# bc-computing/fantoch

Hardware: AMD Instinct MI355X
Metric: executed cmds/sec (node) for batched Atlas/EPaxos sims; % of HBM roofline (higher is better)
Workload: dtype u32

## Files before the change

fantoch_amd/csrc/sim_wave.hip:

```cpp
#include <hip/hip_runtime.h>
#include <stdint.h>

#include <algorithm>
#include <cstdio>
#include <cstring>
#include <vector>

#include "fantoch_amd.h"
#include "fx_internal.h"
#include "fx_synth.h"
#include "fx_wave.h"

namespace fx {
namespace sim {

constexpr uint32_t NMAX = FX_SIM_MAX_N;
constexpr uint32_t CMAX = 32;
constexpr uint32_t KMAX = 2;
constexpr uint32_t VMAX = 16;
constexpr uint32_t FMAX = 12;
constexpr uint32_t RDMAX = 16;
constexpr uint32_t HC_BINS = 64;
constexpr uint32_t HD_BINS = 224;
constexpr uint32_t HMAX = 2;
constexpr uint32_t NONE = 0xFFFFFFFFu;
constexpr uint32_t LNIL = 0xFFFFu;
constexpr uint32_t PT_SEQ = 0, PT_FAST = 8, PT_SLOW = 16, PT_EXEC = 24, PT_OCC = 32, PT_WAIT = 48;

#ifdef FX_SIM_PROFILE
#define PROF_T0() const uint64_t prof_t0_ = __builtin_amdgcn_s_memtime()
#define PROF_ADD(cat) prof[cat] += __builtin_amdgcn_s_memtime() - prof_t0_
#else
#define PROF_T0() (void)0
#define PROF_ADD(cat) (void)0
#endif

enum : uint32_t { M_COLLECT = 0, M_COLLECT_ACK = 1, M_COMMIT = 2, M_CONSENSUS = 3, M_CONSENSUS_ACK = 4,
                  M_COMMIT_DOT = 5, M_GC = 6, M_STABLE = 7,
                  M_STORE = 8, M_STORE_ACK = 9, M_COMMIT_BASIC = 10,
                  M_SUBMIT = 15  };
enum : uint32_t { ST_START = 0, ST_PAYLOAD = 1, ST_COLLECT = 2, ST_COMMIT = 3 };
enum : uint32_t { PH_IDLE = 0, PH_DFS = 1, PH_TRY = 2, PH_CHECK = 3 };

constexpr uint32_t SL_CLIENT = 0,
    SL_IDX = 1, SL_KEYS = 2, SL_PST = 3,
    SL_MASKS = 5, SL_CNT = 6, SL_COLLECT = 7;


struct Geo {
  uint32_t n, C, K, W, R, L, NP, ncli_keys, rt, rc, rdm;
  uint32_t amax, vmax, sl_value, sl_ack, slotw;
  uint32_t off_pool, off_free, off_gct, off_gcc, off_gcr, off_slot, off_kd, off_frame, off_wl, off_hist, words;
};

__host__ __device__ constexpr uint32_t cmin(uint32_t a, uint32_t b) { return a < b ? a : b; }
__host__ __device__ constexpr uint32_t cmax(uint32_t a, uint32_t b) { return a > b ? a : b; }

__host__ __device__ constexpr bool geo_make(uint32_t n, uint32_t C, uint32_t K, uint32_t pool, uint32_t ring,
                                            uint32_t wslots, Geo& g) {
  if (n < 2 || n > NMAX) return false;
  if (C < 1 || C > CMAX) return false;
  g.n = n;
  g.C = C;
  g.K = K;
  const uint32_t cpr = (C + n - 1) / n;
  g.W = wslots ? wslots : (n > 5 && C <= 8 ? 32u : cmin(64u, 8u * C));
  if (g.W > 256u) return false;
  g.R = ring ? ring : cmin(4096u, cmax(16u * n * cpr, n > 5 ? 192u : 0u));
  if (g.R > 65534u) return false;
  g.NP = n * (n - 1);
  g.L = g.NP + n + 2 * C;
  if (g.L > 64 * HMAX) return false;
  g.ncli_keys = pool + C + 1;
  g.amax = 2 * g.K;
  g.vmax = cmin(VMAX, g.K * (n + 1));
  g.sl_value = SL_COLLECT + g.K;
  g.sl_ack = g.sl_value + g.vmax;
  g.slotw = g.sl_ack + n * g.amax;
  if (n * g.amax > 64 || g.slotw > 64) return false;
  uint32_t o = 0;
  g.off_pool = o; o += g.R * 4;
  g.off_free = o; o += g.R;
  g.rt = 4;
  while (g.rt < 4 * cpr && g.rt < 64) g.rt <<= 1;
  if (g.W > 64u) g.rt = cmax(g.rt, 32u);
  g.rc = g.rt / 2;
  g.off_gct = o; o += n * n * g.rt * 2;
  g.off_gcc = o; o += n * n * g.rc * 2;
  if (g.R >= n * n) {
    g.off_gcr = g.off_pool;
  } else {
    g.off_gcr = o; o += n * n * 4;
  }
  g.off_slot = o; o += g.W * g.slotw;
  g.off_kd = o; o += n * g.ncli_keys;
  g.rdm = cmin(RDMAX, C);
  g.off_frame = o; o += FMAX * g.rdm;
  g.off_wl = o; o += 68;
  g.off_hist = o; o += HD_BINS;
  g.words = (o + 3) & ~3u;
  return true;
}
__host__ __device__ constexpr Geo geo_fixed(uint32_t n, uint32_t C) {
  Geo g{};
  geo_make(n, C, 1, 1, 0, 0, g);
  return g;
}

constexpr uint32_t FANY = 0xFFu;
struct GeoRT {
  static constexpr bool fixed = false;
  static constexpr uint32_t proto = 0xFFu, fc = FANY, xp_lanes = 0;
  Geo g;
};
template <uint32_t PR, uint32_t N, uint32_t F, uint32_t CC>
struct GeoCT {
  static constexpr bool fixed = true;
#ifdef FX_XSWAP
  static constexpr uint32_t proto = PR, fc = F, xp_lanes = 0;
#else
  static constexpr uint32_t proto = PR, fc = F, xp_lanes = 64u / N;
#endif
  static constexpr Geo g = geo_fixed(N, CC);
};

struct SimArgs {
  const fx_sim_spec* specs;
  uint32_t instances;
  Geo g;
  const uint16_t* ping;
  const uint8_t* rank;
  uint32_t RP;
  uint32_t exec_cap, lat_cap, max_events, sim_exec_notif;
  uint32_t* executed;
  uint32_t* executed_len;
  uint32_t* latency_log;
  unsigned long long* lat_hist;
  uint32_t lat_bins;
  unsigned long long* chain_hist;
  uint32_t chain_bins;
  unsigned long long* delay_hist;
  uint32_t delay_bins;
  unsigned long long* stats;
  uint32_t* err;
  uint32_t* dot_client;
};

typedef __attribute__((address_space(4))) const SimArgs KSimArgs;
__device__ __forceinline__ KSimArgs* kargs() {
  KSimArgs* p = (KSimArgs*)__builtin_amdgcn_kernarg_segment_ptr();
  asm volatile("" : "+s"(p));
  return p;
}
__device__ __forceinline__ uint32_t vdiv(uint32_t x) {
  uint32_t r;
  asm("v_mov_b32 %0, %1" : "=v"(r) : "v"(x));
  return r;
}

template <uint32_t N>
__device__ __forceinline__ uint32_t rsel(const uint32_t (&a)[N], uint32_t i) {
  uint32_t r = 0;
#pragma unroll
  for (uint32_t k = 0; k < N; ++k) r = (i == k) ? a[k] : r;
  return r;
}
template <uint32_t N>
__device__ __forceinline__ void rput(uint32_t (&a)[N], uint32_t i, uint32_t v) {
#pragma unroll
  for (uint32_t k = 0; k < N; ++k) a[k] = (i == k) ? v : a[k];
}

__device__ __forceinline__ uint32_t tid(uint32_t t) { return t & 127u; }
__device__ __forceinline__ uint32_t tlow(uint32_t t) { return (t >> 7) & 127u; }
__device__ __forceinline__ uint32_t tep(uint32_t t) { return t >> 14; }
__device__ __forceinline__ uint32_t tmk(uint32_t id, uint32_t low, uint32_t ep) { return id | (low << 7) | (ep << 14); }
constexpr uint32_t EPOCH_MAX = 0xFFFFu;

template <uint32_t HM, uint32_t DS, uint32_t NX, class GP>
struct Sim : GP {
  using GP::g;
  uint32_t lid_;
  __device__ __forceinline__ uint32_t lidv() const {
    uint32_t x = lid_;
    asm volatile("" : "+v"(x));
    return x;
  }
  uint32_t* lds;
  uint32_t protocol, n, f, synod_f, fq, wq;
  enum : uint32_t { P_SEED = 0, P_RNG = 2, P_GC = 4, P_EN = 5, P_CMDS = 6, P_CONFLICT = 7, P_POOL = 8, P_EXTRA = 9,
                    P_HAS_EXTRA = 10, P_FINAL = 11, P_CDONE = 12, P_ERRSITE = 13, P_INST = 14,
                    P_F = 15, P_FQ = 16, P_SYNOD_F = 17, P_PROTO = 18, P_OFF_FRAME = 19, P_RDM = 20 };
  uint32_t pv = 0;
  __device__ __forceinline__ uint32_t prm(uint32_t k) const {
    uint32_t r;
    asm volatile("s_nop 1\n\tv_readlane_b32 %0, %1, %2\n\ts_nop 4" : "=s"(r) : "v"(pv), "i"(k));
    return r;
  }
  __device__ __forceinline__ uint64_t prm64(uint32_t k) const {
    return (uint64_t)prm(k) | ((uint64_t)prm(k + 1) << 32);
  }
  __device__ __forceinline__ void prm_set(uint32_t k, uint32_t x) {
    if (lidv() == k) pv = x;
  }
  enum : uint32_t { LG_EXEC = 0, LG_DOTC = 8, LG_LAT = 32 };
  uint64_t lgb = 0;
  uint32_t lgc = 0;
  __device__ __forceinline__ void logs_init(const SimArgs& a, uint32_t inst) {
    const uint32_t l = lidv();
    const bool ex = l < n, dc = (l >= LG_DOTC) & (l - LG_DOTC < n), lt = (l >= LG_LAT) & (l - LG_LAT < g.C);
    const uint64_t prow = (uint64_t)inst * n + (l & 7u), crow = (uint64_t)inst * g.C + (l & 31u);
    const uint64_t be = (uint64_t)a.executed, bd = (uint64_t)a.dot_client, bl = (uint64_t)a.latency_log;
    uint64_t b = 0;
    uint32_t c = 0;
    b = (ex & (be != 0)) ? be + prow * a.exec_cap * 4u : b;
    b = (dc & (bd != 0)) ? bd + prow * a.exec_cap * 4u : b;
    b = (lt & (bl != 0)) ? bl + crow * a.lat_cap * 4u : b;
    c = (ex | dc) ? a.exec_cap : c;
    c = lt ? a.lat_cap : c;
    lgb = b;
    lgc = b != 0 ? c : 0u;
  }
  __device__ __forceinline__ void log_put(uint32_t l, uint32_t table, uint32_t k, uint32_t i, uint32_t v) {
    typedef __attribute__((address_space(1))) uint32_t gu32;
    if ((l - table == k) & (i < lgc)) *(gu32*)(lgb + (uint64_t)i * 4u) = v;
  }
  __device__ __forceinline__ uint32_t proto_() const { if constexpr (GP::fixed) return protocol; else return prm(P_PROTO); }
  __device__ __forceinline__ uint32_t f_() const { if constexpr (GP::fixed) return f; else return prm(P_F); }
  __device__ __forceinline__ uint32_t fq_() const { if constexpr (GP::fixed) return fq; else return prm(P_FQ); }
  __device__ __forceinline__ uint32_t synod_f_() const { if constexpr (GP::fixed) return synod_f; else return prm(P_SYNOD_F); }
  uint32_t C;
  uint32_t err = 0;
  __device__ __forceinline__ void fail_cap(uint32_t line) {
    if (!err) prm_set(P_ERRSITE, line);
    err = FX_ERR_SIM_CAPACITY;
  }
  __device__ __forceinline__ void fail_late(uint32_t line) {
    if (!err) prm_set(P_ERRSITE, line);
    err = FX_ERR_SIM_LATE;
  }
  uint32_t now = 0;
  uint32_t seq = 0;
  uint32_t events = 0;
  uint64_t trace, deps_total, lat_sum;
  uint32_t hcv = 0, hlk = 0, hlc = 0;
  bool done = false, in_extra = false;

  uint32_t ht[HM], hs[HM];
  uint32_t gf = 0, gw = 0, gnt = 0, glk = 0, gkm = 0, gnc = 0;
  uint32_t pt = 0, pq = 0;
  uint32_t ca = 0, cb = 0, cd = 0;
  uint32_t dpq = 0;
  uint32_t frw = 0, frd = 0;
  uint32_t rhv = 0xFFFFFFFFu;
  uint32_t nfree = 0;
  uint32_t sdv[DS];
  uint32_t ecf = 0, ecw = 0;

  uint32_t xdot[NX], xrec[NX], xwait[NX];
  uint32_t sdot, srec, swait, stl, sfr;
  static constexpr bool XSL = GP::xp_lanes != 0;
  uint32_t frow;
  uint64_t occ, wmask, tmask;
  static constexpr uint32_t XPL = GP::xp_lanes;
  uint64_t pmask = ~0ull;
  uint32_t xk, epoch, nwl, phase, root, idc, nfr, missing, fv, fdi, fnc, in_try, emitted, xp;
#ifdef FX_SIM_PROFILE
  uint64_t prof[32] = {};
#endif

  __device__ __forceinline__ uint32_t& W(uint32_t i) { return lds[i]; }
  __device__ __forceinline__ uint32_t& msg(uint32_t e, uint32_t w) {
    return lds[g.off_pool + e * 4 + w];
  }
  __device__ __forceinline__ uint32_t* gct(uint32_t p, uint32_t s) { return &lds[g.off_gct + (p * g.n + s) * g.rt * 2]; }
  __device__ __forceinline__ uint32_t* gcc(uint32_t p, uint32_t s) { return &lds[g.off_gcc + (p * g.n + s) * g.rc * 2]; }
  __device__ __forceinline__ uint32_t* gcr(uint32_t p, uint32_t s) { return &lds[g.off_gcr + (p * g.n + s) * 4]; }
  __device__ __forceinline__ uint32_t slot_find(uint32_t d) const {
    uint32_t r = NONE;
#pragma unroll
    for (uint32_t k = 0; k < DS; ++k) {
      const uint64_t m = bal(sdv[k] == d && d != 0u);
      if (m && r == NONE) r = k * 64u + ctz64(m);
    }
    return r;
  }
  __device__ __forceinline__ void slot_set(uint32_t sl, uint32_t d) {
    const uint32_t l = lidv();
#pragma unroll
    for (uint32_t k = 0; k < DS; ++k) sdv[k] = (((sl >> 6) == k) & (l == (sl & 63u))) ? d : sdv[k];
  }
  __device__ __forceinline__ uint32_t slot_alloc() const {
#pragma unroll
    for (uint32_t k = 0; k < DS; ++k) {
      const uint32_t lo = k * 64u;
      if (lo >= g.W) break;
      const uint64_t pool = g.W - lo >= 64u ? ~0ull : ((1ull << (g.W - lo)) - 1ull);
      const uint64_t fre = ~bal(sdv[k] != 0u) & pool;
      if (fre) return lo + ctz64(fre);
    }
    return NONE;
  }
  __device__ __forceinline__ uint32_t& S(uint32_t sl, uint32_t w) { return lds[g.off_slot + sl * g.slotw + w]; }
  __device__ __forceinline__ uint32_t& kd(uint32_t p, uint32_t key) { return lds[g.off_kd + p * g.ncli_keys + key]; }
  __device__ __forceinline__ uint32_t rdm_() const { if constexpr (GP::fixed) return g.rdm; else return prm(P_RDM); }
  __device__ __forceinline__ uint32_t& FRR(uint32_t fi, uint32_t r) {
    if constexpr (GP::fixed) return lds[g.off_frame + fi * g.rdm + r];
    else return lds[prm(P_OFF_FRAME) + fi * prm(P_RDM) + r];
  }
  __device__ __forceinline__ uint32_t& wl(uint32_t i) { return lds[g.off_wl + i]; }
  __device__ __forceinline__ void hist_chain(uint32_t v) {
    const uint32_t l = lidv();
    if (v < HC_BINS) {
      hcv += l == v ? 1u : 0u;
    } else if (l == 0) {
      KSimArgs* k = kargs();
      if (k->chain_hist) atomicAdd(&k->chain_hist[min(v, k->chain_bins - 1u)], 1ull);
    }
  }
  __device__ __forceinline__ void hist_lat(uint32_t region, uint32_t lat) {
    const uint32_t key = (region << 24) | min(lat, 0xFFFFFFu);
    const uint32_t h = (key * 2654435761u) >> 26;
    const uint32_t k = rl(hlk, h);
    const uint32_t l = lidv();
    if ((k == key + 1u) | (k == 0)) {
      hlk = l == h ? key + 1u : hlk;
      hlc += l == h ? 1u : 0u;
    } else {
      flush_lat(key, 1u);
    }
  }
  __device__ __forceinline__ void flush_lat(uint32_t key, uint32_t cnt) {
    if (lidv() == 0) {
      KSimArgs* k = kargs();
      const uint32_t lat = key & 0xFFFFFFu, bins = k->lat_bins;
      if (k->lat_hist) atomicAdd(&k->lat_hist[(key >> 24) * bins + min(lat, bins - 1u)], (unsigned long long)cnt);
    }
  }
  __device__ __forceinline__ void hist_delay(uint32_t v) {
#ifdef FX_ABL_HIST
    return;
#endif
    const uint32_t l = lidv();
    if (v < HD_BINS) {
      const uint32_t cnt = lds[g.off_hist + v];
      put(lds[g.off_hist + v], cnt + 1u);
    } else if (l == 0) {
      KSimArgs* k = kargs();
      if (k->delay_hist) atomicAdd(&k->delay_hist[min(v, k->delay_bins - 1u)], 1ull);
    }
  }
// ... 496 lines not shown
      if (cl[e * 2] <= x) {
        v = cl[e * 2 + 1];
        return true;
      }
    }
    v = 0;
    return nc <= g.rc;
  }

  __device__ __forceinline__ uint32_t gc_next_after(uint32_t x, uint32_t& pair) {
    const uint32_t gc_ms = prm(P_GC);
    const uint32_t tick = (x / gc_ms + 1u) * gc_ms;
    uint32_t tv = NONE;
    const uint32_t p = lidv() >> 3, q = lidv() & 7u;
    if (p < n && q < n && p != q) {
      const uint32_t d = dpq;
      tv = x < gc_ms + d ? gc_ms + d : ((x - d) / gc_ms + 1u) * gc_ms + d;
    }
    uint32_t tmin = tv;
    for (uint32_t o = 1; o < 64; o <<= 1) tmin = min(tmin, (uint32_t)__shfl_xor((int)tmin, (int)o));
    tmin = uni(tmin);
    if (tick <= tmin) {
      pair = NONE;
      return tick;
    }
    pair = ctz64(bal(tv == tmin));
    return tmin;
  }

  __device__ __forceinline__ void gc_finish(uint32_t tc, uint32_t pair, unsigned long long* st) {
    const uint32_t gc_ms = prm(P_GC);
    if (gc_lane(lidv() >> 3)) {
      uint32_t* r = gcr(lidv() >> 3, lidv() & 7u);
      r[0] = gf;
      r[1] = gnt;
      r[2] = gkm;
      r[3] = gnc;
    }
    for (uint32_t q = 0; q < n; ++q) {
      uint32_t m = 0;
      const bool pl = lidv() < n && lidv() != q;
      const uint32_t dq = gather(dpq, (lidv() * 8u + q) & 63u);
      if (pl) {
        const uint32_t d = dq;
        if (tc > d) m = (tc - d - 1u) / gc_ms;
        if (pair == lidv() * 8u + q && tc >= d + gc_ms && (tc - d) % gc_ms == 0) ++m;
      }
      uint32_t stable = 0;
      if (!bal(pl && m == 0)) {
        uint32_t tl = pl ? m * gc_ms + dq : 0u;
        for (uint32_t o = 1; o < 64; o <<= 1) tl = max(tl, (uint32_t)__shfl_xor((int)tl, (int)o));
        tl = uni(tl);
        uint32_t cur = 0;
        bool ok = true;
        if (lidv() < n) ok = gc_value_at(q, lidv(), tl, cur);
        for (uint32_t p = 0; p < n; ++p) {
          if (p == q) continue;
          const uint32_t kl = rl(m, p) - 1u;
          uint32_t v = 0;
          if (lidv() < n) {
            ok = ok && gc_tick_value(p, lidv(), kl, v);
            cur = min(cur, v);
          }
        }
        if (bal(lidv() < n && !ok)) fail_cap(__LINE__);
        for (uint32_t s2 = 0; s2 < n; ++s2) stable += rl(cur, s2);
      }
      if (st && lidv() == 0) st[FX_SIM_STAT_STABLE + q] = stable;
    }
  }

  __device__ __forceinline__ bool mine(uint64_t m) const {
    return mine(m, lidv());
  }
  __device__ __forceinline__ static bool mine(uint64_t m, uint32_t l) {
    const uint32_t half = l < 32u ? (uint32_t)m : (uint32_t)(m >> 32);
    return (half >> (l & 31u)) & 1u;
  }
  __device__ __forceinline__ uint32_t vcount_of(uint32_t d) { return uni(S(slot_find(d), SL_CNT)) & 0xFFu; }
  __device__ __forceinline__ uint32_t value_at(uint32_t d, uint32_t j) { return uni(S(slot_find(d), g.sl_value + j)); }

  __device__ __forceinline__ void x_load(uint32_t p) {
    xp = p;
    root = idc = nfr = missing = fv = fdi = fnc = in_try = emitted = nwl = 0;
    stl = 0;
    if constexpr (!XSL) sfr = 0;
    frow = 0;
    epoch = 1;
    if constexpr (XPL != 0) {
      pmask = ((1ull << XPL) - 1ull) << (p * XPL);
      occ = bal(sdot != 0u) & pmask;
      wmask = bal(swait != 0u) & pmask;
    } else {
      sdot = rsel(xdot, p); srec = rsel(xrec, p); swait = rsel(xwait, p);
      occ = (uint64_t)rl(pt, PT_OCC + p) | ((uint64_t)rl(pt, PT_OCC + 8u + p) << 32);
      wmask = (uint64_t)rl(pt, PT_WAIT + p) | ((uint64_t)rl(pt, PT_WAIT + 8u + p) << 32);
    }
    xk = rl(pt, PT_EXEC + p);
    tmask = 0;
    phase = PH_IDLE;
  }
  __device__ __forceinline__ void x_store() {
    const uint32_t p = xp;
    if constexpr (XPL != 0) {
      lset(pt, PT_EXEC + p, xk);
      return;
    }
    rput(xdot, p, sdot); rput(xrec, p, srec); rput(xwait, p, swait);
    const uint32_t l = lidv();
    const uint32_t k = (l & 7u) == p ? l >> 3 : NONE;
    pt = k == PT_OCC / 8u ? (uint32_t)occ : pt;
    pt = k == PT_OCC / 8u + 1u ? (uint32_t)(occ >> 32) : pt;
    pt = k == PT_WAIT / 8u ? (uint32_t)wmask : pt;
    pt = k == PT_WAIT / 8u + 1u ? (uint32_t)(wmask >> 32) : pt;
    pt = k == PT_EXEC / 8u ? xk : pt;
  }

  __device__ __forceinline__ bool contains_v(uint32_t d) const {
    const uint32_t si = (d >> FX_SEQ_BITS) - 1u;
    const uint32_t ln = (xp * 8u + si) & 63u;
    const uint32_t fr = gather(ecf, ln), w = gather(ecw, ln);
    const uint32_t sq = d & FX_SEQ_MASK, off = sq - fr - 1u;
    return (si < n) & ((sq <= fr) | ((off < 32u) & (((w >> (off & 31u)) & 1u) != 0u)));
  }
  __device__ __forceinline__ bool contains_u(uint32_t d) const {
    const uint32_t si = (d >> FX_SEQ_BITS) - 1u;
    if (si >= n) return false;
    const uint32_t fr = rl(ecf, xp * 8u + si), w = rl(ecw, xp * 8u + si);
    const uint32_t sq = d & FX_SEQ_MASK, off = sq - fr - 1u;
    return sq <= fr || (off < 32u && ((w >> off) & 1u));
  }
  __device__ __forceinline__ void clk_add(uint32_t d) {
    const uint32_t l = lidv();
    const uint32_t si = (d >> FX_SEQ_BITS) - 1u, sq = d & FX_SEQ_MASK;
    const uint32_t own = si < n ? xp * 8u + si : NONE;
    const uint32_t off = ((l == own) & (sq > ecf)) ? sq - ecf - 1u : NONE;
    if (bal(off + 1u > 32u)) fail_cap(__LINE__);
    ecw |= off - 1u < 31u ? 1u << (off & 31u) : 0u;
    const bool adv = off == 0u;
    const uint32_t win = ecw >> 1;
    const uint32_t ones = __builtin_ctz(~win);
    ecf = adv ? ecf + 1u + ones : ecf;
    ecw = adv ? win >> ones : ecw;
    if (si >= n) err = FX_ERR_DOT_RANGE;
  }
  __device__ __forceinline__ int find(uint32_t d) const {
    const uint64_t m = bal(mine(occ) & (sdot == d));
    return m ? (int)ctz64(m) : -1;
  }
  __device__ __forceinline__ void new_epoch() {
    epoch = epoch + 1;
    if (epoch > EPOCH_MAX) {
      stl = mine(occ) ? tmk(tid(stl), tlow(stl), 0) : stl;
      epoch = 1;
    }
  }

  __device__ __forceinline__ void on_execute(uint32_t d, uint32_t start) {
    const uint32_t sl = slot_find(d);
    if (sl == NONE) { fail_late(__LINE__); return; }
    on_execute_slot(d, start, sl);
  }
  __device__ __forceinline__ void on_execute_slot(uint32_t d, uint32_t start, uint32_t sl) {
    const uint32_t row = slot_row(sl);
    on_execute_at(d, start, sl, rl(row, SL_CLIENT), (rl(row, SL_CNT) >> 20) & 3u, rl(row, SL_MASKS));
  }
  __device__ __forceinline__ void on_execute_at(uint32_t d, uint32_t start, uint32_t sl, uint32_t c, uint32_t nk,
                                                uint32_t masks) {
    const uint32_t p = xp;
    log_put(lidv(), LG_EXEC, p, xk, d);
    ++xk;
    const uint32_t delay = now - start;
    hist_delay(delay);
    if ((rl(ca, c) & 0xFFu) == p) {
      const uint32_t pend = rl(cb, 32u + c);
      if (pend < nk) { fail_late(__LINE__); return; }
      lset(cb, 32u + c, pend - nk);
      if (pend == nk) {
        const uint32_t w = fw_(), nr = (w >> 20) & 31u;
        if (nr >= rdm_()) { fail_cap(__LINE__); return; }
        put(FRR(nfrm - 1, nr), c);
        fw_set(w + (1u << 20));
      }
    }
    if (((masks >> 24) & 0xFFu) + 1u == n) {
      slot_set(sl, 0u);
    } else {
      put(S(sl, SL_MASKS), masks + (1u << 24));
    }
  }

  __device__ __forceinline__ void emit_one(uint32_t d, uint32_t start, uint32_t sl, uint32_t c, uint32_t nk, uint32_t masks) {
    hist_chain(1u);
    clk_add(d);
    on_execute_at(d, start, sl, c, nk, masks);
  }

  __device__ __forceinline__ int insert_vertex(uint32_t d, uint32_t dsl) {
    const uint64_t fre = ~occ & pmask;
    if (!fre) { fail_cap(__LINE__); return -1; }
    const uint32_t sl = ctz64(fre);
    const bool me = lidv() == sl;
    sdot = me ? d : sdot;
    srec = me ? now : srec;
    swait = me ? 0u : swait;
    stl = me ? 0u : stl;
    if constexpr (XSL) sfr = me ? dsl << 16 : sfr;
    occ |= 1ull << sl;
    return (int)sl;
  }

  __device__ __forceinline__ void frame_vertex(uint32_t v) {
    fv = v;
    if constexpr (XSL) {
      frow = slot_row(rl(sfr, v) >> 16);
      fnc = rl(frow, SL_CNT) & 0xFFu;
    } else {
      fnc = vcount_of(rl(sdot, v));
    }
  }
  __device__ __forceinline__ void dfs_start(uint32_t r, bool intry) {
    root = r;
    in_try = intry;
    emitted = 0;
    missing = 0;
    idc = 1;
    const uint32_t tr = rl(stl, r);
    stl = lidv() == r ? tmk(1, 1, tep(tr)) : stl;
    nfr = 0;
    fdi = 0;
    frame_vertex(r);
    phase = PH_DFS;
  }

  __device__ __forceinline__ void save_scc() {
    const uint32_t idv = tid(rl(stl, fv));
    const uint32_t l = lidv();
    const uint32_t myid = tid(stl);
    const bool mem = mine(occ, l) & (myid >= idv);
    const uint64_t mm = bal(mem);
    const uint32_t cnt = pop64(mm);
    if (nwl + cnt > 65u) { fail_cap(__LINE__); return; }
    hist_chain(cnt);
    uint32_t rank = 0;
    for (uint64_t m = mm; m; m &= m - 1) rank += rl(sdot, ctz64(m)) < sdot ? 1u : 0u;
    for (uint32_t r = 0; r < cnt; ++r) {
      const uint32_t lr = ctz64(bal(mem & (rank == r)));
      const uint32_t d = rl(sdot, lr);
      const uint32_t st = rl(srec, lr);
      put(wl(nwl + r), d);
      clk_add(d);
      if constexpr (XSL) on_execute_slot(d, st, rl(sfr, lr) >> 16);
      else on_execute(d, st);
      if (err) return;
    }
    nwl += cnt;
    if constexpr (XPL != 0) {
      sdot = mem ? 0u : sdot;
      swait = mem ? 0u : swait;
    }
    occ &= ~mm;
    wmask &= ~mm;
    tmask &= ~mm;
    emitted = 1;
  }

  __device__ __forceinline__ void dfs_finish() {
    const bool mark = in_try && missing != 0 && !emitted;
    const uint32_t l = lidv();
    const uint32_t myid = tid(stl);
    stl = (mine(occ, l) & (myid != 0)) ? tmk(0, 0, mark ? epoch : tep(stl)) : stl;
    if (missing) {
      swait = l == root ? missing : swait;
      wmask |= 1ull << root;
    }
    if (in_try) {
      if (!missing || emitted) new_epoch();
      phase = PH_TRY;
    } else {
      phase = PH_CHECK;
    }
  }

  __device__ __forceinline__ void dfs_iter() {
    const uint32_t l = lidv();
    if (fdi < fnc) {
      const uint32_t vd = rl(sdot, fv);
      const uint32_t dep = XSL ? rl(frow, g.sl_value + fdi) : value_at(vd, fdi);
      ++fdi;
      if (dep == vd || contains_u(dep)) return;
      const int x = find(dep);
      if (x < 0) {
        missing = dep;
        dfs_finish();
        return;
      }
      const uint32_t tx = rl(stl, (uint32_t)x);
      if (tid(tx) == 0) {
        ++idc;
        if (idc > 127u) { fail_cap(__LINE__); return; }
        stl = l == (uint32_t)x ? tmk(idc, idc, tep(tx)) : stl;
        sfr = l == nfr ? (XSL ? sfr & 0xFFFF0000u : 0u) | fv | (fdi << 8) : sfr;
        ++nfr;
        fdi = 0;
        frame_vertex((uint32_t)x);
      } else {
        const uint32_t tv = rl(stl, fv);
        stl = ((tid(tx) < tlow(tv)) & (l == fv)) ? tmk(tid(tv), tid(tx), tep(tv)) : stl;
      }
    } else {
      const uint32_t tv = rl(stl, fv);
      const uint32_t lowv = tlow(tv);
      if (tid(tv) == lowv) {
        save_scc();
        if (err) return;
      }
      if (nfr == 0) {
        dfs_finish();
        return;
      }
      --nfr;
      const uint32_t fw = rl(sfr, nfr);
      fdi = (fw >> 8) & 0xFFu;
      frame_vertex(fw & 0xFFu);
      const uint32_t tp = rl(stl, fv);
      stl = ((lowv < tlow(tp)) & (l == fv)) ? tmk(tid(tp), lowv, tep(tp)) : stl;
    }
  }

  __device__ __forceinline__ void try_iter() {
    if (!tmask) { phase = PH_CHECK; return; }
    uint32_t best = ctz64(tmask), best_dot = rl(sdot, best);
    for (uint64_t m = tmask & (tmask - 1); m; m &= m - 1) {
      const uint32_t b = ctz64(m), v = rl(sdot, b);
      if (v < best_dot) {
        best_dot = v;
        best = b;
      }
    }
    tmask &= ~(1ull << best);
    if (tep(rl(stl, best)) == epoch) return;
    dfs_start(best, true);
  }

  __device__ __forceinline__ void check_iter() {
    if (nwl == 0 || !wmask) {
      nwl = 0;
      phase = PH_IDLE;
      return;
    }
    --nwl;
    const uint32_t x = uni(wl(nwl));
    const uint32_t l = lidv();
    const uint64_t t = bal(mine(wmask, l) & (swait == x));
    if (!t) return;
    wmask &= ~t;
    if constexpr (XPL != 0) {
      swait = mine(t, l) ? 0u : swait;
    }
    tmask = t;
    new_epoch();
    phase = PH_TRY;
  }

  __device__ __forceinline__ void x_add(uint32_t p, uint32_t d, uint32_t dsl, uint32_t depj) {
    PROF_T0();
    x_load(p);
    nwl = 0;
    if (find(d) >= 0) { err = FX_ERR_DOUBLE_INDEX; x_store(); return; }
    const uint32_t hcnt = rl(depj, SL_CNT), vc = hcnt & 0xFFu;
    const uint32_t hcli = rl(depj, SL_CLIENT), hmasks = rl(depj, SL_MASKS);
    deps_total += vc;
    const uint32_t l = lidv();
    const bool exd = contains_v(depj);
    const bool keep = (l - g.sl_value < vc) & (depj != d) & !exd;
    PROF_ADD(5);
    if (!bal(keep)) {
#ifdef FX_SIM_PROFILE
      const uint64_t pe0 = __builtin_amdgcn_s_memtime();
#endif
      emit_one(d, now, dsl, hcli, (hcnt >> 20) & 3u, hmasks);
#ifdef FX_SIM_PROFILE
      prof[13] += __builtin_amdgcn_s_memtime() - pe0;
      prof[21] += 1;
#endif
      if (wmask && !err) {
        put(wl(0), d);
        nwl = 1;
        phase = PH_CHECK;
      }
    } else {
      put(S(dsl, SL_MASKS), hmasks);
      const int sl = insert_vertex(d, dsl);
      if (sl >= 0) dfs_start((uint32_t)sl, false);
    }
    uint32_t guard = 0;
    while (phase != PH_IDLE && !err && ++guard <= (1u << 22)) {
      if (phase == PH_DFS) dfs_iter();
      else if (phase == PH_TRY) try_iter();
      else check_iter();
    }
    if (guard > (1u << 22)) fail_cap(__LINE__);
#ifdef FX_SIM_PROFILE
    const uint64_t ps0 = __builtin_amdgcn_s_memtime();
#endif
    x_store();
#ifdef FX_SIM_PROFILE
    prof[14] += __builtin_amdgcn_s_memtime() - ps0;
    prof[22] += 1;
#endif
  }

  __device__ __forceinline__ void frame_push() {
    fw = 0;
    fd = 0;
    if (nfrm >= FMAX) { fail_cap(__LINE__); return; }
    ++nfrm;
    if constexpr (!FIH) lset(frw, nfrm - 1, 0);
    xinfo = 0;
    xsl = 0;
    xrow = 0;
  }

  __device__ __forceinline__ void run_handlers(uint32_t p, uint32_t from, uint32_t kind, uint32_t w2) {
    PROF_T0();
    run_handlers_(p, from, kind, w2);
    PROF_ADD(7);
  }
  __device__ __forceinline__ void run_handlers_(uint32_t p, uint32_t from, uint32_t kind, uint32_t w2) {
    bool pend = true;
    while ((pend || nfrm != 0) && !err) {
#ifndef FX_HOIST_P
      asm volatile("s_nop 1\n\tv_readfirstlane_b32 %0, %1\n\ts_nop 4" : "=s"(p) : "v"(p));
#endif
#ifdef FX_SIM_PROFILE
      prof[24] += 1;
#endif
      if (pend) {
        pend = false;
        frame_push();
        if (!err) {
          PROF_T0();
          switch (kind) {
            case M_SUBMIT: h_submit(p, w2); break;
            case M_COLLECT: h_mcollect(p, from, w2); break;
            case M_COLLECT_ACK: h_mcollectack(p, from, w2); break;
            case M_COMMIT: h_mcommit(p, from, w2); break;
            case M_CONSENSUS: h_mconsensus(p, from, w2); break;
            case M_CONSENSUS_ACK: h_mconsensusack(p, from, w2); break;
            default:
              if constexpr (!GP::fixed) {
                if (kind == M_STORE) { h_mstore(p, from, w2); break; }
                if (kind == M_STORE_ACK) { h_mstoreack(p, from, w2); break; }
                if (kind == M_COMMIT_BASIC) { h_bcommit(p, w2); break; }
              }
              err = FX_ERR_INVALID_ARG;
          }
#ifdef FX_SIM_PROFILE
          prof[8 + min(kind, 7u)] += __builtin_amdgcn_s_memtime() - prof_t0_;
          prof[16 + min(kind, 7u)] += 1;
#endif
          if (xinfo && !err) {
            const uint32_t d = xinfo;
            xinfo = 0;
            PROF_T0();
            x_add(p, d, xsl, xrow);
            PROF_ADD(2);
          }
        }
      } else if constexpr (FIH) {
        fw = rl(frw, nfrm - 1);
        fd = rl(frd, nfrm - 1);
      }
      if (!err) {
        PROF_T0();
        const uint32_t fi = nfrm - 1;
        const uint32_t w = fw_(), dot = fd_();
        if (w & 3u) {
          const uint32_t tgt = (w >> 8) & 0xFFu, k2 = (w >> 2) & 15u;
          const uint32_t nx = (w >> 16) & 15u;
          const bool self = ((tgt >> p) & 1u) && p >= nx;
          const uint32_t hi = self ? p : n;
          send_batch(p, tgt & ((1u << hi) - 1u) & ~((1u << nx) - 1u) & ~(1u << p), k2, dot);
          if (self && !err) {
// ... 228 lines not shown
        const uint32_t k = a.rank[rc * RP + sp.process_regions[p]];
        if (k < bk) {
          bk = k;
          best = p;
        }
      }
      for (uint32_t i = 0; i < sp.clients_per_region; ++i, ++c) {
        if (s.lidv() == c) {
          s.ca = best | (rc << 8);
          s.cd = a.ping[rc * RP + sp.process_regions[best]] / 2u;
        }
        if (s.lidv() == 32u + c) s.cd = a.ping[sp.process_regions[best] * RP + rc] / 2u;
      }
    }
  }
  __builtin_amdgcn_s_barrier();
  const bool sim_en = a.sim_exec_notif || has_extra;
  for (uint32_t p = 0; p < n; ++p) {
    if (sim_en) s.schedule_timer(s.link_e(p), en_ms);
    else ++s.seq;
  }
  s.logs_init(a, inst);
  for (uint32_t c = 0; c < s.C; ++c) {
    s.client_send(c);
    if (sp.commands_per_client == 0) s.err = FX_ERR_INVALID_ARG;
  }
  const uint32_t max_events = a.max_events ? a.max_events : 0xFFFFFFFFu;
  uint32_t gc_pair = NONE;
  while (!s.done && !s.err) {
    uint32_t t = 0;
#ifdef FX_SIM_PROFILE
    const uint64_t pt0 = __builtin_amdgcn_s_memtime();
#endif
    const uint32_t link = s.pop_min(t);
#ifdef FX_SIM_PROFILE
    const uint64_t pt1 = __builtin_amdgcn_s_memtime();
    s.prof[0] += pt1 - pt0;
#endif
    if (link == NONE || t == NONE) {
      s.err = FX_ERR_SIM_LATE;
      break;
    }
    if (t < s.now) {
      s.err = FX_ERR_TIME_RANGE;
      break;
    }
    if (s.in_extra && t > s.prm(s.P_FINAL) && gc_ms) {
      uint32_t pair = NONE;
      const uint32_t tg = s.gc_next_after(s.prm(s.P_FINAL), pair);
      if (tg < t) {
        s.now = tg;
        gc_pair = pair;
        break;
      }
    }
    s.now = t;
    s.run_event(link);
#ifdef FX_SIM_PROFILE
    s.prof[1] += __builtin_amdgcn_s_memtime() - pt1;
#endif
    if (s.in_extra && s.now > s.prm(s.P_FINAL)) s.done = true;
    if (s.events >= max_events) s.err = FX_ERR_SIM_EVENTS;
  }
  __builtin_amdgcn_s_barrier();
  const uint32_t o_exec = gather(s.pt, (PT_EXEC + s.lidv()) & 63u), o_fast = gather(s.pt, (PT_FAST + s.lidv()) & 63u),
                 o_slow = gather(s.pt, (PT_SLOW + s.lidv()) & 63u);
  if (s.lidv() < n && a.executed_len) a.executed_len[(size_t)inst * n + s.lidv()] = o_exec;
  if (a.stats) {
    unsigned long long* st = a.stats + (size_t)inst * FX_SIM_STATS;
    if (s.lidv() < NMAX) {
      const bool v = s.lidv() < n;
      st[FX_SIM_STAT_FAST + s.lidv()] = v ? o_fast : 0u;
      st[FX_SIM_STAT_SLOW + s.lidv()] = v ? o_slow : 0u;
      st[FX_SIM_STAT_STABLE + s.lidv()] = 0u;
      st[FX_SIM_STAT_FAST_READS + s.lidv()] = 0u;
      st[FX_SIM_STAT_SLOW_READS + s.lidv()] = 0u;
    }
    if (gc_ms && !s.err) s.gc_finish(s.now, gc_pair, st);
    const uint32_t err_site = s.prm(s.P_ERRSITE);
    if (s.lidv() == 0) {
      st[FX_SIM_STAT_EVENTS] = s.events;
#ifdef FX_SIM_PROFILE
      for (uint32_t i = 0; i < 24; ++i) st[i] = s.prof[i];
      for (uint32_t i = 24; i < 32; ++i) st[FX_SIM_STAT_FAST_READS + i - 24u] = s.prof[i];
#endif
      st[FX_SIM_STAT_END_MS] = s.now;
      st[FX_SIM_STAT_TRACE] = s.trace;
      st[FX_SIM_STAT_SEQ] = s.seq;
      st[FX_SIM_STAT_DEPS] = s.deps_total;
      st[FX_SIM_STAT_LAT_SUM] = s.lat_sum;
      st[FX_SIM_STAT_ERR_SITE] = err_site;
    }
  }
  if (s.hcv && a.chain_hist) atomicAdd(&a.chain_hist[min(s.lidv(), a.chain_bins - 1u)], (unsigned long long)s.hcv);
  for (uint32_t i = s.lidv(); i < HD_BINS; i += 64) {
    const uint32_t c = smem[s.g.off_hist + i];
    if (c && a.delay_hist) atomicAdd(&a.delay_hist[min(i, a.delay_bins - 1u)], (unsigned long long)c);
  }
  if (s.hlk && a.lat_hist) {
    const uint32_t key = s.hlk - 1u, lat = key & 0xFFFFFFu;
    atomicAdd(&a.lat_hist[(key >> 24) * a.lat_bins + min(lat, a.lat_bins - 1u)], (unsigned long long)s.hlc);
  }
  if (s.lidv() == 0) a.err[inst] = s.err;
}

}

using namespace sim;

size_t simx_arena_bytes(const fx_sim_spec& sp, uint32_t ring, uint32_t dots);
bool simx_table_sizes(const fx_sim_spec& sp, uint32_t ring, uint32_t dots, uint32_t* R, uint32_t* NS);
int simx_launch(const fx_sim_batch* b, const fx_sim_output* o, hipStream_t hs);

using GeoC1 = GeoCT<FX_PROTOCOL_EPAXOS, 5, 2, 5>;
#ifdef FX_XSWAP
constexpr uint32_t XNX = 5;
#else
constexpr uint32_t XNX = 1;
#endif
using GeoC0 = GeoCT<FX_PROTOCOL_ATLAS, 3, 1, 3>;
using GeoC2a = GeoCT<FX_PROTOCOL_ATLAS, 5, FANY, 5>;
using GeoC2b = GeoCT<FX_PROTOCOL_ATLAS, 7, FANY, 7>;
template <class GP>
static bool geo_is(const Geo& g, const fx_sim_spec& s0) {
  const Geo c = GP::g;
  return s0.protocol == GP::proto && (GP::fc == FANY || s0.f == GP::fc) && std::memcmp(&g, &c, sizeof(Geo)) == 0;
}

static bool sim_geometry(const fx_sim_spec& sp, uint32_t ring, uint32_t wslots, Geo& g) {
  return geo_make(sp.n, sp.clients_per_region * sp.num_client_regions, sp.keys_per_command, sp.pool_size, ring,
                  wslots, g);
}

}

using namespace fx;

extern "C" {

int fx_sim_plan(const fx_sim_spec* sp, uint32_t ring_entries, uint32_t dot_slots, uint32_t* lds_bytes) {
  if (!sp || !lds_bytes) return FX_ERR_INVALID_ARG;
  Geo g;
  if (!sim_geometry(*sp, ring_entries, dot_slots, g)) return FX_ERR_UNSUPPORTED;
  *lds_bytes = g.words * 4;
  return FX_OK;
}

int fx_sim_plan_large(const fx_sim_spec* sp, uint32_t ring_entries, uint32_t dot_slots, uint64_t* arena_bytes) {
  if (!sp || !arena_bytes) return FX_ERR_INVALID_ARG;
  const size_t b = simx_arena_bytes(*sp, ring_entries, dot_slots);
  if (!b) return FX_ERR_UNSUPPORTED;
  *arena_bytes = b;
  return FX_OK;
}

int fx_sim_run(const fx_sim_batch* b, const fx_sim_output* o, void* hip_stream) {
  if (!b || !o || !b->specs || !b->host_specs || !o->err || !b->planet_ping || !b->planet_rank) return FX_ERR_INVALID_ARG;
  if (b->instances == 0) return FX_OK;
  int dc = 0;
  if (hipGetDeviceCount(&dc) != hipSuccess || dc <= 0) return FX_ERR_NO_DEVICE;
  const uint32_t ring = b->ring_entries;
  const uint32_t W = b->dot_slots;
  if (ring > 65534 || W > 8u * 65536u) return FX_ERR_INVALID_ARG;
  const fx_sim_spec& s0 = b->host_specs[0];
  bool large = (b->flags & FX_SIM_FLAG_LARGE) != 0 || W > 256;
  bool one_p = true, one_f = true;
  for (uint32_t i = 0; i < b->instances; ++i) {
// ... 284 lines not shown
```

Baseline: 640.4 million.

## Skip already-executed deps via keep bitmask and seed DFS from first missing dep

Adds a per-frame bitmask of dependencies still worth visiting (not self, not executed), so DFS iterations jump straight to the next live dependency instead of stepping through and discarding filtered entries one per iteration. On insertion of a new vertex, the keep ballot already computed is reused: if the first live dependency is absent, the vertex is parked directly in the wait set without running a DFS; otherwise the DFS starts at that dependency. Extra profiling counters are added under the profile flag. The change increases register state (fk) and adds ballot work in frame_vertex, and it only applies to fixed-geometry instances with n<=5 when FX_SEARCH_ROOT is at least 2.

```diff
diff --git a/fantoch_amd/csrc/sim_wave.hip b/fantoch_amd/csrc/sim_wave.hip
--- a/fantoch_amd/csrc/sim_wave.hip
+++ b/fantoch_amd/csrc/sim_wave.hip
@@ -30,9 +30,17 @@
 #ifdef FX_SIM_PROFILE
 #define PROF_T0() const uint64_t prof_t0_ = __builtin_amdgcn_s_memtime()
 #define PROF_ADD(cat) prof[cat] += __builtin_amdgcn_s_memtime() - prof_t0_
+#define PROF_LO(i) prof[i] += 1ull
+#define PROF_HI(i) prof[i] += 1ull << 32
 #else
 #define PROF_T0() (void)0
 #define PROF_ADD(cat) (void)0
+#define PROF_LO(i) (void)0
+#define PROF_HI(i) (void)0
+#endif
+
+#ifndef FX_SEARCH_ROOT
+#define FX_SEARCH_ROOT 2
 #endif
 
 enum : uint32_t { M_COLLECT = 0, M_COLLECT_ACK = 1, M_COMMIT = 2, M_CONSENSUS = 3, M_CONSENSUS_ACK = 4,
@@ -111,6 +119,7 @@
 struct GeoRT {
   static constexpr bool fixed = false;
   static constexpr uint32_t proto = 0xFFu, fc = FANY, xp_lanes = 0;
+  static constexpr bool jump = false;
   Geo g;
 };
 template <uint32_t PR, uint32_t N, uint32_t F, uint32_t CC>
@@ -121,6 +130,7 @@
 #else
   static constexpr uint32_t proto = PR, fc = F, xp_lanes = 64u / N;
 #endif
+  static constexpr bool jump = N <= 5;
   static constexpr Geo g = geo_fixed(N, CC);
 };
 
@@ -260,13 +270,16 @@
   uint32_t xdot[NX], xrec[NX], xwait[NX];
   uint32_t sdot, srec, swait, stl, sfr;
   static constexpr bool XSL = GP::xp_lanes != 0;
+  static constexpr bool JUMP = XSL && GP::jump && FX_SEARCH_ROOT >= 2;
   uint32_t frow;
   uint64_t occ, wmask, tmask;
   static constexpr uint32_t XPL = GP::xp_lanes;
   uint64_t pmask = ~0ull;
   uint32_t xk, epoch, nwl, phase, root, idc, nfr, missing, fv, fdi, fnc, in_try, emitted, xp;
+  uint32_t fk;
 #ifdef FX_SIM_PROFILE
-  uint64_t prof[32] = {};
+  uint64_t prof[40] = {};
+  uint32_t pclean = 0;
 #endif
 
   __device__ __forceinline__ uint32_t& W(uint32_t i) { return lds[i]; }
@@ -929,7 +942,7 @@
 
   __device__ __forceinline__ void x_load(uint32_t p) {
     xp = p;
-    root = idc = nfr = missing = fv = fdi = fnc = in_try = emitted = nwl = 0;
+    root = idc = nfr = missing = fv = fdi = fnc = fk = in_try = emitted = nwl = 0;
     stl = 0;
     if constexpr (!XSL) sfr = 0;
     frow = 0;
@@ -1062,11 +1075,17 @@
     if constexpr (XSL) {
       frow = slot_row(rl(sfr, v) >> 16);
       fnc = rl(frow, SL_CNT) & 0xFFu;
+      if constexpr (JUMP) fk = row_keep(frow, fnc, rl(sdot, v));
     } else {
       fnc = vcount_of(rl(sdot, v));
     }
   }
-  __device__ __forceinline__ void dfs_start(uint32_t r, bool intry) {
+  __device__ __forceinline__ uint32_t row_keep(uint32_t row, uint32_t cnt, uint32_t vd) const {
+    const bool exd = contains_v(row);
+    const bool keep = (lidv() - g.sl_value < cnt) & (row != vd) & !exd;
+    return (uint32_t)(bal(keep) >> g.sl_value);
+  }
+  __device__ __forceinline__ void dfs_begin(uint32_t r, bool intry) {
     root = r;
     in_try = intry;
     emitted = 0;
@@ -1076,8 +1095,15 @@
     stl = lidv() == r ? tmk(1, 1, tep(tr)) : stl;
     nfr = 0;
     fdi = 0;
+    phase = PH_DFS;
+#ifdef FX_SIM_PROFILE
+    pclean = 1;
+#endif
+  }
+  __device__ __forceinline__ void dfs_start(uint32_t r) {
+    PROF_HI(32);
+    dfs_begin(r, true);
     frame_vertex(r);
-    phase = PH_DFS;
   }
 
   __device__ __forceinline__ void save_scc() {
@@ -1131,17 +1157,37 @@
 
   __device__ __forceinline__ void dfs_iter() {
     const uint32_t l = lidv();
-    if (fdi < fnc) {
-      const uint32_t vd = rl(sdot, fv);
-      const uint32_t dep = XSL ? rl(frow, g.sl_value + fdi) : value_at(vd, fdi);
-      ++fdi;
-      if (dep == vd || contains_u(dep)) return;
+    if (JUMP ? fk != 0u : fdi < fnc) {
+      uint32_t dep;
+      if constexpr (JUMP) {
+        fdi = (uint32_t)__builtin_ctz(fk);
+        fk &= fk - 1u;
+        dep = rl(frow, g.sl_value + fdi);
+        ++fdi;
+#ifdef FX_SIM_PROFILE
+        if (contains_u(dep)) PROF_LO(37);
+#endif
+      } else {
+        const uint32_t vd = rl(sdot, fv);
+        dep = XSL ? rl(frow, g.sl_value + fdi) : value_at(vd, fdi);
+        ++fdi;
+        if (dep == vd || contains_u(dep)) {
+          PROF_HI(33);
+          return;
+        }
+      }
       const int x = find(dep);
       if (x < 0) {
+#ifdef FX_SIM_PROFILE
+        if (pclean) { if (in_try) PROF_LO(36); else PROF_LO(35); }
+#endif
         missing = dep;
         dfs_finish();
         return;
       }
+#ifdef FX_SIM_PROFILE
+      pclean = 0;
+#endif
       const uint32_t tx = rl(stl, (uint32_t)x);
       if (tid(tx) == 0) {
         ++idc;
@@ -1156,6 +1202,10 @@
         stl = ((tid(tx) < tlow(tv)) & (l == fv)) ? tmk(tid(tv), tid(tx), tep(tv)) : stl;
       }
     } else {
+#ifdef FX_SIM_PROFILE
+      if (pclean && in_try) PROF_HI(35);
+      pclean = 0;
+#endif
       const uint32_t tv = rl(stl, fv);
       const uint32_t lowv = tlow(tv);
       if (tid(tv) == lowv) {
@@ -1170,6 +1220,7 @@
       const uint32_t fw = rl(sfr, nfr);
       fdi = (fw >> 8) & 0xFFu;
       frame_vertex(fw & 0xFFu);
+      if constexpr (JUMP) fk &= ~0u << fdi;
       const uint32_t tp = rl(stl, fv);
       stl = ((lowv < tlow(tp)) & (l == fv)) ? tmk(tid(tp), lowv, tep(tp)) : stl;
     }
@@ -1187,7 +1238,7 @@
     }
     tmask &= ~(1ull << best);
     if (tep(rl(stl, best)) == epoch) return;
-    dfs_start(best, true);
+    dfs_start(best);
   }
 
   __device__ __forceinline__ void check_iter() {
@@ -1237,16 +1288,52 @@
         phase = PH_CHECK;
       }
     } else {
+      PROF_LO(32);
       put(S(dsl, SL_MASKS), hmasks);
       const int sl = insert_vertex(d, dsl);
-      if (sl >= 0) dfs_start((uint32_t)sl, false);
+      if constexpr (FX_SEARCH_ROOT == 0) {
+        if (sl >= 0) {
+          dfs_begin((uint32_t)sl, false);
+          frame_vertex((uint32_t)sl);
+        }
+      } else if (sl >= 0) {
+        const uint64_t km = bal(keep);
+        const uint32_t fl = ctz64(km);
+        const uint32_t dep = rl(depj, fl);
+        if (find(dep) < 0) {
+          PROF_LO(35);
+          swait = l == (uint32_t)sl ? dep : swait;
+          wmask |= 1ull << sl;
+        } else {
+          dfs_begin((uint32_t)sl, false);
+          fv = (uint32_t)sl;
+          fnc = vc;
+          fdi = fl - g.sl_value;
+          if constexpr (XSL) frow = depj;
+          if constexpr (JUMP) fk = (uint32_t)(km >> g.sl_value);
+          if (fdi) PROF_HI(36);
+        }
+      }
     }
     uint32_t guard = 0;
+#ifdef FX_SIM_PROFILE
+    const uint64_t pl0 = __builtin_amdgcn_s_memtime();
+    const bool pin = phase != PH_IDLE;
+    if (pin) PROF_HI(37);
+#endif
     while (phase != PH_IDLE && !err && ++guard <= (1u << 22)) {
+#ifdef FX_SIM_PROFILE
+      if (phase == PH_DFS) PROF_LO(33);
+      else if (phase == PH_TRY) PROF_LO(34);
+      else PROF_HI(34);
+#endif
       if (phase == PH_DFS) dfs_iter();
       else if (phase == PH_TRY) try_iter();
       else check_iter();
     }
+#ifdef FX_SIM_PROFILE
+    if (pin) prof[38] += __builtin_amdgcn_s_memtime() - pl0;
+#endif
     if (guard > (1u << 22)) fail_cap(__LINE__);
 #ifdef FX_SIM_PROFILE
     const uint64_t ps0 = __builtin_amdgcn_s_memtime();
@@ -1641,7 +1728,7 @@
       st[FX_SIM_STAT_EVENTS] = s.events;
 #ifdef FX_SIM_PROFILE
       for (uint32_t i = 0; i < 24; ++i) st[i] = s.prof[i];
-      for (uint32_t i = 24; i < 32; ++i) st[FX_SIM_STAT_FAST_READS + i - 24u] = s.prof[i];
+      for (uint32_t i = 24; i < 40; ++i) st[FX_SIM_STAT_FAST_READS + i - 24u] = s.prof[i];
 #endif
       st[FX_SIM_STAT_END_MS] = s.now;
       st[FX_SIM_STAT_TRACE] = s.trace;
```

Measured after the change: 661.8 million (median of 6 runs). 3.3% higher.
